# wdmwhh/MRefSR

Measured on AMD Instinct MI355X. Metric: 4x SR Mpix/sec, 5-ref 160x160->640x640; PSNR within 0.01 dB of ref, higher is better.
Workload: dtype f32

## Files before the change

mrefsr_amd/csrc/conv_wino4.hip:

```cpp
#include <cstdlib>
#include <type_traits>

#include "conv_wino_common.h"

namespace {
using namespace mrefsr_conv;
using namespace mrefsr_wino;

constexpr int NSLOT = 2;
constexpr int SLOT_BYTES = RAW_BYTES;
constexpr int RING_OFF = 0;
constexpr int RING_BYTES = 4 * 4 * 4096;
constexpr int X_LD = 32 + 4;
constexpr int X_BYTES = 4 * NTILE * X_LD * 4;
constexpr int SLOT_OFF = RING_OFF + RING_BYTES;
constexpr int BIAS_OFF = SLOT_OFF + NSLOT * SLOT_BYTES;
constexpr int SINK_OFF = BIAS_OFF + BIAS_MAX * 4;
constexpr int X_OFF = SINK_OFF + 256 * 16;
constexpr int LDS_BYTES = X_OFF + X_BYTES;
static_assert(LDS_BYTES <= 160 * 1024 && (RING_OFF & 4095) == 0 && (SLOT_OFF & 15) == 0 && (X_OFF & 15) == 0, "conv_wino4: LDS budget");
constexpr int NPD = 6, PROWS = 3;
static_assert(NPD * PROWS == PP && PROWS * PP * 4 <= 256, "conv_wino4: patch piece assignment");
constexpr unsigned int OOB = 0xffff0000u;

__device__ __forceinline__ f32x16 mma16(const u32x4 a, const u32x4 b, const f32x16 c)
{
    return __builtin_amdgcn_mfma_f32_32x32x16_f16(__builtin_bit_cast(f16x8, a), __builtin_bit_cast(f16x8, b), c, 0, 0, 0);
}

template <int I, int N, class F> __device__ __forceinline__ void sfor(F &&f)
{
    if constexpr (I < N) {
        f(std::integral_constant<int, I>{});
        sfor<I + 1, N>(f);
    }
}

__device__ __forceinline__ void bload16(f32x4 &dst, const unsigned int voff, const __amdgpu_buffer_rsrc_t srd, const unsigned int soff)
{
    asm volatile("s_nop 4\n\tbuffer_load_dwordx4 %0, %1, %2, %3 offen" : "=v"(dst) : "v"(voff), "s"(srd), "s"(soff) : "memory");
}
template <int N> __device__ __forceinline__ void vm_wait_p(f32x4 (&p)[NPD])
{
    asm volatile("s_waitcnt vmcnt(%6)" : "+v"(p[0]), "+v"(p[1]), "+v"(p[2]), "+v"(p[3]), "+v"(p[4]), "+v"(p[5]) : "n"(N) : "memory");
}
__device__ __forceinline__ void dma_group(const unsigned int m0v, const unsigned int voff, const void *sbase)
{
    asm volatile("s_mov_b32 m0, %0\n\ts_nop 0\n\tglobal_load_lds_dwordx4 %1, %2\n\tglobal_load_lds_dwordx4 %1, %2 offset:1024\n\t"
                 "global_load_lds_dwordx4 %1, %2 offset:2048\n\tglobal_load_lds_dwordx4 %1, %2 offset:3072"
                 : : "s"(m0v), "v"(voff), "s"(sbase) : "memory");
}
template <int OFF> __device__ __forceinline__ void dma_frag(const unsigned int m0v, const unsigned int voff, const void *sbase)
{
    if constexpr (OFF == 0)
        asm volatile("s_mov_b32 m0, %0\n\ts_nop 0\n\tglobal_load_lds_dwordx4 %1, %2" : : "s"(m0v), "v"(voff), "s"(sbase) : "memory");
    else
        asm volatile("global_load_lds_dwordx4 %0, %1 offset:%2" : : "v"(voff), "s"(sbase), "n"(OFF) : "memory");
}
template <int N> __device__ __forceinline__ void vm_wait() { asm volatile("s_waitcnt vmcnt(%0)" : : "n"(N) : "memory"); }

struct TState {
    f32x4 a[4], b[4], t[4], v[4];
};
template <int K>
__device__ __forceinline__ void top(TState &s, const unsigned char *const pa, const unsigned char *const pb, const float sr, u32x4 (&vh)[4], u32x4 (&vl)[4])
{
    constexpr int g0 = (K < 24 || (K >= 32 && K < 72)) ? 0 : 1;
    if constexpr (K < 8 || (K >= 24 && K < 32)) {
        constexpr int r = K < 8 ? K : K - 24, c = r >> 1;
        constexpr int co = ((c & 1) * RAW_CP + (c >> 1)) * 16 + g0 * (RAW_Q * 16);
        if constexpr (r & 1) s.b[c] = *reinterpret_cast<const f32x4 *>(pb + co);
        else s.a[c] = *reinterpret_cast<const f32x4 *>(pa + co);
    } else if constexpr ((K >= 8 && K < 24) || (K >= 72 && K < 88)) {
        constexpr int r = K < 24 ? K - 8 : K - 72, c = r >> 2, e = r & 3;
        s.t[c][e] = __builtin_fmaf(sr, s.b[c][e], s.a[c][e]);
    } else if constexpr ((K >= 32 && K < 48) || (K >= 88 && K < 104)) {
        constexpr int r = K < 48 ? K - 32 : K - 88, j = r >> 2, e = r & 3;
        if constexpr (j == 0) s.v[0][e] = s.t[0][e] - s.t[2][e];
        else if constexpr (j == 1) s.v[1][e] = s.t[1][e] + s.t[2][e];
        else if constexpr (j == 2) s.v[2][e] = s.t[2][e] - s.t[1][e];
        else s.v[3][e] = s.t[1][e] - s.t[3][e];
    } else {
        constexpr int r = K < 72 ? K - 48 : K - 104, u = r / 3, sub = r % 3, j = u >> 1, p = u & 1, w = 2 * g0 + p;
        if constexpr (sub == 0) vh[j][w] = pk_f16(s.v[j][2 * p], s.v[j][2 * p + 1]);
        else if constexpr (sub == 1) {
            unsigned int lo;
            asm("v_fma_mixlo_f16 %0, %1, -1.0, %2 op_sel_hi:[1,0,0]" : "=v"(lo) : "v"(vh[j][w]), "v"(s.v[j][2 * p]));
            vl[j][w] = lo;
        } else {
            unsigned int lo = vl[j][w];
            asm("v_fma_mixhi_f16 %0, %1, -1.0, %2 op_sel:[1,0,0] op_sel_hi:[1,0,0]" : "+v"(lo) : "v"(vh[j][w]), "v"(s.v[j][2 * p + 1]));
            vl[j][w] = lo;
        }
    }
}
constexpr int QA[24] = {4, 4, 6, 6, 6, 6, 5, 6, 5, 6, 6, 6, 4, 5, 4, 5, 5, 5, 5, 6, 5, 6, 6, 6};
constexpr int QB[24] = {4, 4, 5, 6, 6, 5, 5, 6, 5, 6, 6, 5, 5, 6, 5, 6, 6, 5, 5, 6, 5, 6, 5, 5};
constexpr int qsum(const int (&q)[24], const int n)
{
    int t = 0;
    for (int i = 0; i < n; ++i) t += q[i];
    return t;
}
static_assert(qsum(QA, 24) == 128 && qsum(QB, 24) == 128, "conv_wino4: every micro-operation of a transform is dealt exactly once");

#ifdef WINO_STAMP
constexpr int NSTAMP = 12;
__device__ unsigned long long g_wino4_stamp[1024][NSTAMP];
#define W4STAMP(i)                                                     \
    {                                                                 \
        const unsigned long long t_now = __builtin_readcyclecounter(); \
        st_acc[i] += t_now - t_last;                                  \
        t_last = t_now;                                               \
    }
#else
#define W4STAMP(i) {}
#endif

#ifndef W4_ABL
#define W4_ABL 0
#endif

template <int RES, bool NT, bool POOL, bool SCALED>
__global__ __launch_bounds__(256, 1) void conv_wino4_kernel(const ConvArgs A)
{
#ifdef WINO_STAMP
    unsigned long long st_acc[NSTAMP] = {0, 0, 0, 0, 0, 0, 0, 0, 0, 0, 0, 0}, t_last = __builtin_readcyclecounter();
#endif
    extern __shared__ __align__(16) unsigned char smem[];
    const int tid = threadIdx.x, lane = tid & 63, wi = __builtin_amdgcn_readfirstlane(tid >> 6);
    const int l31 = lane & 31, kh = lane >> 5;
    const int H = A.H, W = A.W;
    const int tiles_x = W / (2 * TT), tiles_y = H / (2 * TT);
    const int n_tiles = A.n_cb * tiles_x * tiles_y * A.wino_N, per = (n_tiles + 7) >> 3;
    const int band0 = (blockIdx.x & 7) * per, band1 = min(band0 + per, n_tiles), tstep = gridDim.x >> 3;
    int tile = band0 + (blockIdx.x >> 3);
    if (tile >= band1) return;
    for (int i = tid; i < A.n_cb * NB; i += 256)
        reinterpret_cast<float *>(smem + BIAS_OFF)[i] = (A.bias && i < A.Cout) ? A.bias[i] : 0.f;
    struct Tile { int n, cb, y0, x0; };
    auto decode = [&](const int lin) {
        Tile t;
        t.cb = lin % A.n_cb;
        int r = lin / A.n_cb;
        t.x0 = (r % tiles_x) * (2 * TT);
        r /= tiles_x;
        t.y0 = (r % tiles_y) * (2 * TT);
        t.n = r / tiles_y;
        return t;
    };
    const int n_ch = A.n_ch;

    f32x16 acc[4][2][2];

    f32x4 pf[NPD];
    const int p_q = tid & 3, p_py = (tid >> 2) / PP, p_px = (tid >> 2) - p_py * PP;
    const bool p_have = tid < PROWS * PP * 4;
    const unsigned int praw0 = p_have ? (unsigned int)(SLOT_OFF + (p_q * RAW_Q + p_py * RAW_RS + (p_px & 1) * RAW_CP + (p_px >> 1)) * 16) : (unsigned int)(SINK_OFF + tid * 16);
    const unsigned int praw_step = p_have ? (unsigned int)(PROWS * RAW_RS * 16) : 0u, praw_slot = p_have ? (unsigned int)SLOT_BYTES : 0u;
    Tile nxt = {0, 0, 0, 0};
    int rq_tile = tile, rq_ch = 0, rq_run = 0;
    int t_n = 0, t_y0 = 0, t_x0 = 0;
    __amdgpu_buffer_rsrc_t rq_srd = __builtin_amdgcn_make_buffer_rsrc(const_cast<float *>(A.x1), 0, 0, 0x00020000);
    unsigned int rq_soff = 0, rq_vo[NPD];
#pragma unroll
    for (int k = 0; k < NPD; ++k) rq_vo[k] = OOB;
    auto prepare = [&]() {
        const bool edge = rq_run == 0;
        const bool wrap = edge && rq_ch == n_ch;
        rq_tile += wrap ? tstep : 0;
        const int ch = wrap ? 0 : rq_ch;
        rq_ch = ch + 1;
        int run = rq_run - 1;
        unsigned int soff = rq_soff + KC * 4;
        if (edge) {
            if (ch == 0) {
                nxt = decode(rq_tile < band1 ? rq_tile : band0);
                t_n = rq_tile < band1 ? nxt.n : -1, t_y0 = nxt.y0, t_x0 = nxt.x0;
            }
            const bool first = ch < A.n_ch1;
            const int cl = first ? ch : ch - A.n_ch1, Cs = first ? A.C1 : A.C2;
            soff = (unsigned int)(cl * KC * 4);
            const int ld = first ? A.ld1 : A.ld2, nn = t_n < 0 ? 0 : t_n;
            const float *const img = first ? A.x1 + (size_t)(nn % A.N1) * H * W * A.ld1 : A.x2 + (size_t)(nn % A.N2) * H * W * A.ld2;
            const unsigned int bytes = __builtin_amdgcn_readfirstlane((unsigned int)((size_t)H * W * ld * 4));
            rq_srd = __builtin_amdgcn_make_buffer_rsrc(const_cast<void *>(scalar_ptr(img)), 0, bytes, 0x00020000);
            const int gy0 = t_y0 + p_py - 1, gx = t_x0 + p_px - 1;
            const bool cok = p_have & (t_n >= 0) & ((unsigned int)gx < (unsigned int)W) & (cl * KC + 4 * p_q < Cs);
            const unsigned int base = ((unsigned int)(gy0 * W + gx) * (unsigned int)ld + 4u * p_q) * 4u;
            const unsigned int step3 = (unsigned int)(PROWS * W * ld) * 4u;
#pragma unroll
            for (int k = 0; k < NPD; ++k)
                rq_vo[k] = (cok & ((unsigned int)(gy0 + k * PROWS) < (unsigned int)H)) ? base + (unsigned int)k * step3 : OOB;
            const int full = Cs / KC;
            run = cl < full ? full - 1 - cl : 0;
        }
        rq_run = __builtin_amdgcn_readfirstlane(run);
        rq_soff = __builtin_amdgcn_readfirstlane(soff);
    };
    auto request_piece = [&](const int k) { bload16(pf[k], rq_vo[k], rq_srd, __builtin_amdgcn_readfirstlane(rq_soff)); };
    float in_s = 1.f, oscale_in = A.out_scale;
    if constexpr (SCALED) {
        const float am = *A.in_amax;
        if (am > 1.0e-30f && am < 3.0e38f) {
            int e;
            (void)frexpf(am, &e);
            in_s = ldexpf(1.f, 12 - e);
            oscale_in = A.out_scale * ldexpf(1.f, e - 12);
        }
        in_s = __uint_as_float(__builtin_amdgcn_readfirstlane(__float_as_uint(in_s)));
    }
    auto store_piece = [&](const int slot, const int k) {
        f32x4 v = pf[k];
        if constexpr (SCALED) v[0] *= in_s, v[1] *= in_s, v[2] *= in_s, v[3] *= in_s;
        *reinterpret_cast<f32x4 *>(smem + praw0 + slot * praw_slot + k * praw_step) = v;
    };

    const int t_ra = wi == 0 ? 0 : (wi == 2 ? 2 : 1), t_rb = wi == 0 ? 2 : (wi == 1 ? 2 : (wi == 2 ? 1 : 3));
    const float t_sr = __uint_as_float(__builtin_amdgcn_readfirstlane(wi == 1 ? 0x3f800000u : 0xbf800000u));
    const unsigned int t_base = (unsigned int)(SLOT_OFF + ((2 * kh) * RAW_Q + (2 * (l31 >> 3)) * RAW_RS + (l31 & 7)) * 16);
    const unsigned int t_a = t_base + t_ra * RAW_RS * 16, t_b = t_base + t_rb * RAW_RS * 16;

    const unsigned int u_voff = (unsigned int)(l31 * KC + kh * 8) * 2u;
    const unsigned short *const u_wave = A.wp + (size_t)(wi * 4) * 2 * NB * KC;
    const unsigned int ring_w = (unsigned int)(RING_OFF + wi * 16384);
    const unsigned char *const frag_l = smem + ring_w + lane * 16;
    int uq_tile = tile, uq_left = 0;
    const unsigned char *u_s = nullptr;
    auto frag_cursor = [&]() {
        const bool edge = uq_left == 0;
        const unsigned char *nb = u_s + WCH_HALVES * 2;
        if (edge) {
            nb = reinterpret_cast<const unsigned char *>(scalar_ptr(u_wave + (size_t)nxt.cb * n_ch * WCH_HALVES));
        }
        u_s = nb;
        uq_tile += edge ? tstep : 0;
        uq_left = edge ? n_ch - 1 : uq_left - 1;
    };
    auto frag_dma = [&](const int j) { dma_group(ring_w + j * 4096, u_voff, u_s + j * 4096); };
    auto frag_dma1 = [&](const int j, auto pc) { dma_frag<decltype(pc)::value * 1024>(ring_w + j * 4096, u_voff, u_s + j * 4096); };
    auto frag_read = [&](const int j, const int ct, const int plane) {
        if constexpr (W4_ABL == 8) return u32x4{(unsigned int)(j + ct), (unsigned int)plane, 0x3c003c00u, 0x3c003c00u};
        else return *reinterpret_cast<const u32x4 *>(frag_l + j * 4096 + plane * 2048 + ct * 1024);
    };

    int sl = 0;
    prepare();
    Tile cur = nxt;
#pragma unroll
    for (int k = 0; k < NPD; ++k) request_piece(k);
    prepare();
    frag_cursor();
    vm_wait_p<0>(pf);
#pragma unroll
    for (int k = 0; k < NPD; ++k) store_piece(0, k);
#pragma unroll
    for (int k = 0; k < NPD; ++k) request_piece(k);
#pragma unroll
    for (int j = 0; j < 4; ++j) frag_dma(j);
    prepare();
    frag_cursor();
    __syncthreads();
    vm_wait_p<12>(pf);
    const float slope = __uint_as_float(__builtin_amdgcn_readfirstlane(__float_as_uint(!A.act ? 1.0f : A.slope_ptr ? *A.slope_ptr : A.slope)));
    u32x4 a0h[4], a0l[4];
    {
        TState ts;
        const unsigned char *const pa = smem + t_a, *const pb = smem + t_b;
        sfor<0, 128>([&](auto kc) { top<decltype(kc)::value>(ts, pa, pb, t_sr, a0h, a0l); });
    }
    float nonfin = 0.f;
    float oamx = 0.f;
    u32x4 ul[2], uh[2];
    ul[0] = frag_read(0, 0, 1), ul[1] = frag_read(0, 1, 1);

    auto step = [&](auto first_c) {
        constexpr bool first = decltype(first_c)::value;
        asm volatile("; W4MARK step_begin");
        u32x4 b1h[4], b1l[4];
        const int sl1 = sl ^ 1;
        {
            TState ts;
            const unsigned char *const pa = smem + t_a + sl * SLOT_BYTES + 8 * RAW_RS * 16;
            const unsigned char *const pb = smem + t_b + sl * SLOT_BYTES + 8 * RAW_RS * 16;
            sfor<0, 24>([&](auto mc) {
                constexpr int m = decltype(mc)::value, j = m / 6, k = m % 6, ct = k & 1, prod = k >> 1;
                if constexpr (m == 0) W4STAMP(0)
                if constexpr (m == 6) W4STAMP(1)
                if constexpr (m == 12) W4STAMP(2)
                if constexpr (m == 18) W4STAMP(3)
                if constexpr (k == 0) uh[0] = frag_read(j, 0, 0), uh[1] = frag_read(j, 1, 0);
                if constexpr (W4_ABL != 4) {
                    f32x16 z;
#pragma unroll
                    for (int e = 0; e < 16; ++e) z[e] = 0.f;
                    if constexpr (prod == 0) acc[j][0][ct] = mma16(ul[ct], a0h[j], first ? z : acc[j][0][ct]);
                    else if constexpr (prod == 1) acc[j][0][ct] = mma16(uh[ct], a0l[j], acc[j][0][ct]);
                    else acc[j][0][ct] = mma16(uh[ct], a0h[j], acc[j][0][ct]);
                } else {
                    asm volatile("" : : "v"(prod == 0 ? ul[ct] : uh[ct]), "v"(prod == 1 ? a0l[j] : a0h[j]));
                }
                if constexpr (W4_ABL != 3) sfor<qsum(QA, m), qsum(QA, m + 1)>([&](auto kc) { top<decltype(kc)::value>(ts, pa, pb, t_sr, b1h, b1l); });
                if constexpr (W4_ABL != 2 && W4_ABL != 7 && m >= 6 && m < 12) store_piece(sl1, m - 6);
                if constexpr (k == 4) {
                    if constexpr (j == 0) vm_wait<8>();
                    if constexpr (j == 1) vm_wait<4>();
                    if constexpr (j == 2) vm_wait<4>();
                    constexpr int jn = j == 3 ? 0 : j + 1;
                    ul[0] = frag_read(jn, 0, 1), ul[1] = frag_read(jn, 1, 1);
                }
                if constexpr (W4_ABL != 2 && W4_ABL != 7 && m >= 12 && m < 18) request_piece(m - 12);
                __builtin_amdgcn_sched_barrier(0);
            });
        }
        W4STAMP(4)
        {
            TState ts;
            const unsigned char *const pa = smem + t_a + sl1 * SLOT_BYTES;
            const unsigned char *const pb = smem + t_b + sl1 * SLOT_BYTES;
            sfor<0, 24>([&](auto mc) {
                constexpr int m = decltype(mc)::value, j = m / 6, k = m % 6, ct = k & 1, prod = k >> 1;
                if constexpr (k == 0) uh[0] = frag_read(j, 0, 0), uh[1] = frag_read(j, 1, 0);
                if constexpr (W4_ABL != 4) {
                    f32x16 z;
#pragma unroll
                    for (int e = 0; e < 16; ++e) z[e] = 0.f;
                    if constexpr (prod == 0) acc[j][1][ct] = mma16(ul[ct], b1h[j], first ? z : acc[j][1][ct]);
                    else if constexpr (prod == 1) acc[j][1][ct] = mma16(uh[ct], b1l[j], acc[j][1][ct]);
                    else acc[j][1][ct] = mma16(uh[ct], b1h[j], acc[j][1][ct]);
                } else {
                    asm volatile("" : : "v"(prod == 0 ? ul[ct] : uh[ct]), "v"(prod == 1 ? b1l[j] : b1h[j]));
                }
                if constexpr (m == 0) {
                    if constexpr (W4_ABL != 6) __syncthreads();
                    W4STAMP(5)
                    __builtin_amdgcn_sched_barrier(0);
                }
                if constexpr (m == 12) W4STAMP(6)
                if constexpr (W4_ABL != 3) sfor<qsum(QB, m), qsum(QB, m + 1)>([&](auto kc) { top<decltype(kc)::value>(ts, pa, pb, t_sr, a0h, a0l); });
                if constexpr (k == 4 && j < 3) ul[0] = frag_read(j + 1, 0, 1), ul[1] = frag_read(j + 1, 1, 1);
                if constexpr (m == 22) {
                    vm_wait_p<10>(pf);
                    ul[0] = frag_read(0, 0, 1), ul[1] = frag_read(0, 1, 1);
                }
                if constexpr (W4_ABL != 1 && W4_ABL != 7 && k >= 2) frag_dma1(j, std::integral_constant<int, k - 2>{});
                __builtin_amdgcn_sched_barrier(0);
            });
        }
        asm volatile("; W4MARK step_cursors");
        W4STAMP(7)
        prepare();
        frag_cursor();
        sl = sl1;
        asm volatile("; W4MARK step_end");
        W4STAMP(8)
    };

    for (;;) {
        const int tile_n = tile + tstep;
        const bool more = tile_n < band1;
        W4STAMP(10)
        step(std::true_type{});
        for (int s = 1; s < n_ch; ++s) step(std::false_type{});

        asm volatile("; W4MARK fast_begin");
        const int cb = cur.cb, n = cur.n, y0 = cur.y0, x0 = cur.x0;
        float *const xb = reinterpret_cast<float *>(smem + X_OFF);
        const int Cout = A.Cout;
        const float oscale = oscale_in;
        int tid_e = tid;
        asm volatile("" : "+v"(tid_e));
        const int c4 = (tid_e & 7) * 4, T0 = tid_e >> 3;
        float *const xrow0 = xb + ((size_t)wi * NTILE + (tid_e & 31)) * X_LD + 4 * ((tid_e >> 5) & 1);
        auto rd = [](const float &a) {
            float v;
            asm volatile("v_accvgpr_read_b32 %0, %1" : "=v"(v) : "a"(a));
            return v;
        };
        auto publish = [&](const int hc, const int b) {
#pragma unroll
            for (int t = 0; t < 2; ++t) {
                float *const xrow = xrow0 + t * 32 * X_LD;
#pragma unroll
                for (int qd = 0; qd < 4; ++qd) {
                    float z[4];
#pragma unroll
                    for (int r = 0; r < 4; ++r) {
                        const int e = 4 * qd + r;
                        if (b == 0) {
                            const float m0 = rd(acc[0][t][hc][e]), m1 = rd(acc[1][t][hc][e]), m2 = rd(acc[2][t][hc][e]);
                            z[r] = m0 + m1 + m2;
                        } else {
                            const float m1 = rd(acc[1][t][hc][e]), m2 = rd(acc[2][t][hc][e]), m3 = rd(acc[3][t][hc][e]);
                            z[r] = m1 + (-m2 - m3);
                        }
                    }
                    *reinterpret_cast<float4 *>(xrow + 8 * qd) = make_float4(z[0], z[1], z[2], z[3]);
                }
            }
        };
        auto gather = [&](const int T, float4 (&y)[2]) {
            float4 z[4];
#pragma unroll
            for (int i = 0; i < 4; ++i) z[i] = *reinterpret_cast<const float4 *>(xb + ((size_t)i * NTILE + T) * X_LD + c4);
            y[0] = make_float4(z[0].x + z[1].x + z[2].x, z[0].y + z[1].y + z[2].y, z[0].z + z[1].z + z[2].z, z[0].w + z[1].w + z[2].w);
            y[1] = make_float4(z[1].x - z[2].x - z[3].x, z[1].y - z[2].y - z[3].y, z[1].z - z[2].z - z[3].z, z[1].w - z[2].w - z[3].w);
        };
        {
            constexpr bool pooled = POOL;
            const int Ho = pooled ? H >> 1 : H, Wo = pooled ? W >> 1 : W, yo = pooled ? y0 >> 1 : y0, xo = pooled ? x0 >> 1 : x0;
            const int ld_r = RES == 2 ? Cout : A.ld_res;
            const __amdgpu_buffer_rsrc_t srd_o = __builtin_amdgcn_make_buffer_rsrc(
                const_cast<void *>(scalar_ptr(A.out + ((size_t)(n * Ho + yo) * Wo + xo) * A.ld_out + cb * NB)), 0, 0xffffffffu, 0x00020000);
            const float *const rbase = RES == 1 ? A.residual + ((size_t)(n * H + y0) * W + x0) * ld_r + cb * NB
                                     : RES == 2 ? A.pre + ((size_t)((n % A.pre_N) * H + y0) * W + x0) * ld_r + cb * NB : A.out;
            const __amdgpu_buffer_rsrc_t srd_r = __builtin_amdgcn_make_buffer_rsrc(const_cast<void *>(scalar_ptr(rbase)), 0, 0xffffffffu, 0x00020000);
            const int pstep = pooled ? 1 : 2;
            const unsigned int vo_o = (unsigned int)(((pstep * (T0 >> 3)) * Wo + pstep * (T0 & 7)) * A.ld_out + c4) * 4u;
            const unsigned int vo_r = (unsigned int)(((2 * (T0 >> 3)) * W + 2 * (T0 & 7)) * ld_r + c4) * 4u;
            const unsigned int row_o = (unsigned int)(Wo * A.ld_out) * 4u, row_r = (unsigned int)(W * ld_r) * 4u;
            constexpr int aux = NT ? 2 : 0;
            if constexpr (W4_ABL == 5) {
#pragma unroll
                for (int j = 0; j < 4; ++j)
#pragma unroll
                    for (int t = 0; t < 4; ++t) nonfin = __builtin_fmaf(rd(acc[j][t >> 1][t & 1][0]), 0.f, nonfin);
            }
#pragma unroll
            for (int hc = 0; hc < (W4_ABL == 5 ? 0 : 2); ++hc) {
                const float4 bv = *reinterpret_cast<const float4 *>(smem + BIAS_OFF + (cb * NB + hc * 32 + c4) * 4);
                float4 pool[2];
#pragma unroll
                for (int b = 0; b < 2; ++b) {
                    if (hc | b) __syncthreads();
                    f32x4 rq[2][2];
                    if constexpr (RES != 0) {
#pragma unroll
                        for (int it = 0; it < 2; ++it)
#pragma unroll
                            for (int a = 0; a < 2; ++a) {
                                const unsigned int so = (unsigned int)(8 * it + a) * row_r + (unsigned int)(b * ld_r + hc * 32) * 4u;
                                rq[it][a] = __builtin_bit_cast(f32x4, __builtin_amdgcn_raw_buffer_load_b128(srd_r, vo_r, so, aux));
                            }
                    }
                    publish(hc, b);
                    __syncthreads();
#pragma unroll
                    for (int it = 0; it < 2; ++it) {
                        __builtin_amdgcn_sched_barrier(0);
                        float4 y[2];
                        gather(T0 + 32 * it, y);
                        if constexpr (pooled) {
                            nonfin = __builtin_fmaf(y[0].x + y[1].x, 0.f, nonfin);
                            float4 m = make_float4(fmaxf(y[0].x, y[1].x), fmaxf(y[0].y, y[1].y), fmaxf(y[0].z, y[1].z), fmaxf(y[0].w, y[1].w));
                            if (b == 0) {
                                pool[it] = m;
                            } else {
                                m = make_float4(fmaxf(m.x, pool[it].x), fmaxf(m.y, pool[it].y), fmaxf(m.z, pool[it].z), fmaxf(m.w, pool[it].w));
                                float4 v = make_float4(m.x * oscale + bv.x, m.y * oscale + bv.y, m.z * oscale + bv.z, m.w * oscale + bv.w);
                                nonfin = __builtin_fmaf(v.x, 0.f, nonfin);
                                v.x = v.x > 0.f ? v.x : v.x * slope, v.y = v.y > 0.f ? v.y : v.y * slope;
                                v.z = v.z > 0.f ? v.z : v.z * slope, v.w = v.w > 0.f ? v.w : v.w * slope;
                                const unsigned int so = (unsigned int)(4 * it) * row_o + (unsigned int)(hc * 32) * 4u;
                                oamx = fmaxf(fmaxf(fmaxf(oamx, fabsf(v.x)), fabsf(v.y)), fmaxf(fabsf(v.z), fabsf(v.w)));
                                __builtin_amdgcn_raw_buffer_store_b128(__builtin_bit_cast(u32x4, f32x4{v.x, v.y, v.z, v.w}), srd_o, vo_o, so, aux);
                            }
                        } else {
#pragma unroll
                            for (int a = 0; a < 2; ++a) {
                                float4 v = y[a];
                                v.x = v.x * oscale + bv.x, v.y = v.y * oscale + bv.y, v.z = v.z * oscale + bv.z, v.w = v.w * oscale + bv.w;
                                nonfin = __builtin_fmaf(v.x, 0.f, nonfin);
                                if constexpr (RES == 2) v.x += rq[it][a][0], v.y += rq[it][a][1], v.z += rq[it][a][2], v.w += rq[it][a][3];
                                v.x = v.x > 0.f ? v.x : v.x * slope, v.y = v.y > 0.f ? v.y : v.y * slope;
                                v.z = v.z > 0.f ? v.z : v.z * slope, v.w = v.w > 0.f ? v.w : v.w * slope;
                                if constexpr (RES == 1) v.x += rq[it][a][0], v.y += rq[it][a][1], v.z += rq[it][a][2], v.w += rq[it][a][3];
                                const unsigned int so = (unsigned int)(8 * it + a) * row_o + (unsigned int)(b * A.ld_out + hc * 32) * 4u;
                                oamx = fmaxf(fmaxf(fmaxf(oamx, fabsf(v.x)), fabsf(v.y)), fmaxf(fabsf(v.z), fabsf(v.w)));
                                __builtin_amdgcn_raw_buffer_store_b128(__builtin_bit_cast(u32x4, f32x4{v.x, v.y, v.z, v.w}), srd_o, vo_o, so, aux);
                            }
                        }
                    }
                }
            }
        }
        asm volatile("; W4MARK fast_end");
        W4STAMP(9)
        if (!more) break;
        tile = tile_n;
        cur = nxt;
    }
    vm_wait_p<0>(pf);
#pragma unroll
    for (int k = 0; k < NPD; ++k) asm volatile("" ::"v"(pf[k]) : "memory");
#pragma unroll
    for (int j = 0; j < 4; ++j) asm volatile("" ::"v"(a0h[j]), "v"(a0l[j]) : "memory");
    if (A.range_flag && !(nonfin == nonfin)) atomicOr(A.range_flag, 1);
    if (A.stat_amax) {
#pragma unroll
        for (int o = 32; o > 0; o >>= 1) oamx = fmaxf(oamx, __shfl_xor(oamx, o, 64));
        if (lane == 0 && oamx > 0.f && oamx < 3.0e38f && __float_as_uint(oamx) > __builtin_nontemporal_load(A.stat_amax)) atomicMax(A.stat_amax, __float_as_uint(oamx));
    }
#ifdef WINO_STAMP
    W4STAMP(10)
    st_acc[11] = 1;
    if (lane == 0)
        for (int i = 0; i < NSTAMP; ++i) atomicAdd(&g_wino4_stamp[(blockIdx.x * 4 + wi) & 1023][i], st_acc[i]);
#endif
}

}

namespace mrefsr_conv {

bool wino4_serves(const ConvArgs &a)
{
    if ((a.H & 15) || (a.W & 15) || (a.Cout & 63) || (a.ld_out & 3) || (a.ld1 & 3) || (a.C1 & 3) || (a.x2 && ((a.ld2 & 3) || (a.C2 & 3)))) return false;
    if (a.epilogue == 1) return !a.residual && !a.pre;
    if (a.epilogue != 0) return false;
    if (a.residual && a.pre) return false;
    if (a.residual && (a.ld_res & 3)) return false;
    return true;
}

int wino4_launch(const ConvArgs &b, int blocks_cu, hipStream_t stream)
{
    const int res = b.residual ? 1 : b.pre ? 2 : 0;
    const bool pool = b.epilogue == 1, nt = b.stream_out != 0;
    const bool sc = b.in_amax != nullptr;
    using K = void (*)(const ConvArgs);
    static const K table[4][2][2] = {
        {{conv_wino4_kernel<0, false, false, false>, conv_wino4_kernel<0, false, false, true>},
         {conv_wino4_kernel<0, true, false, false>, conv_wino4_kernel<0, true, false, true>}},
        {{conv_wino4_kernel<1, false, false, false>, conv_wino4_kernel<1, false, false, true>},
         {conv_wino4_kernel<1, true, false, false>, conv_wino4_kernel<1, true, false, true>}},
        {{conv_wino4_kernel<2, false, false, false>, conv_wino4_kernel<2, false, false, true>},
         {conv_wino4_kernel<2, true, false, false>, conv_wino4_kernel<2, true, false, true>}},
        {{conv_wino4_kernel<0, false, true, false>, conv_wino4_kernel<0, false, true, true>},
         {conv_wino4_kernel<0, true, true, false>, conv_wino4_kernel<0, true, true, true>}}};
    const int ki = pool ? 3 : res;
    const K kern = table[ki][nt ? 1 : 0][sc ? 1 : 0];
    static unsigned long long attr[16] = {0, 0, 0, 0, 0, 0, 0, 0, 0, 0, 0, 0, 0, 0, 0, 0};
    if (mrefsr::first_use_on_device(attr[(ki * 2 + (nt ? 1 : 0)) * 2 + (sc ? 1 : 0)]))
        (void)hipFuncSetAttribute(reinterpret_cast<const void *>(kern), hipFuncAttributeMaxDynamicSharedMemorySize, LDS_BYTES);
    hipLaunchKernelGGL(kern, dim3(blocks_cu), dim3(256), LDS_BYTES, stream, b);
    return mrefsr::check_launch("conv_wino4");
}

}

#ifdef WINO_STAMP
MREFSR_EXPORT int mrefsr_dbg_wino4_stamps(unsigned long long *out12)
{
    static unsigned long long h[1024][NSTAMP];
    if (hipDeviceSynchronize() != hipSuccess) return mrefsr::fail(MREFSR_E_LAUNCH, "wino4_stamps: sync failed");
    if (hipMemcpyFromSymbol(h, HIP_SYMBOL(g_wino4_stamp), sizeof(h)) != hipSuccess) return mrefsr::fail(MREFSR_E_LAUNCH, "wino4_stamps: read failed");
    for (int i = 0; i < NSTAMP; ++i) out12[i] = 0;
    for (int s = 0; s < 1024; ++s)
        for (int i = 0; i < NSTAMP; ++i) out12[i] += h[s][i], h[s][i] = 0;
    if (hipMemcpyToSymbol(HIP_SYMBOL(g_wino4_stamp), h, sizeof(h)) != hipSuccess) return mrefsr::fail(MREFSR_E_LAUNCH, "wino4_stamps: reset failed");
    return 0;
}
#endif
```

Before: 16.19.

## Software-pipeline Winograd output epilogue: precompute column folds and prefetch residuals

Restructures the epilogue of the Winograd conv kernel. The AGPR reads and column fold for the next half-channel group are computed while the current group's LDS gather is in flight, and residual loads are issued one phase ahead. The aim is to hide AGPR-read, LDS and global-load latency behind the barrier-separated publish/gather phases. The cost is more live VGPRs for the prefolded values and prefetched residuals, which may raise register pressure or cause spills.

```diff
diff --git a/mrefsr_amd/csrc/conv_wino4.hip b/mrefsr_amd/csrc/conv_wino4.hip
--- a/mrefsr_amd/csrc/conv_wino4.hip
+++ b/mrefsr_amd/csrc/conv_wino4.hip
@@ -367,7 +367,6 @@
         const int cb = cur.cb, n = cur.n, y0 = cur.y0, x0 = cur.x0;
         float *const xb = reinterpret_cast<float *>(smem + X_OFF);
         const int Cout = A.Cout;
-        const float oscale = oscale_in;
         int tid_e = tid;
         asm volatile("" : "+v"(tid_e));
         const int c4 = (tid_e & 7) * 4, T0 = tid_e >> 3;
@@ -377,34 +376,22 @@
             asm volatile("v_accvgpr_read_b32 %0, %1" : "=v"(v) : "a"(a));
             return v;
         };
-        auto publish = [&](const int hc, const int b) {
-#pragma unroll
-            for (int t = 0; t < 2; ++t) {
-                float *const xrow = xrow0 + t * 32 * X_LD;
-#pragma unroll
-                for (int qd = 0; qd < 4; ++qd) {
-                    float z[4];
-#pragma unroll
-                    for (int r = 0; r < 4; ++r) {
-                        const int e = 4 * qd + r;
-                        if (b == 0) {
-                            const float m0 = rd(acc[0][t][hc][e]), m1 = rd(acc[1][t][hc][e]), m2 = rd(acc[2][t][hc][e]);
-                            z[r] = m0 + m1 + m2;
-                        } else {
-                            const float m1 = rd(acc[1][t][hc][e]), m2 = rd(acc[2][t][hc][e]), m3 = rd(acc[3][t][hc][e]);
-                            z[r] = m1 + (-m2 - m3);
-                        }
-                    }
-                    *reinterpret_cast<float4 *>(xrow + 8 * qd) = make_float4(z[0], z[1], z[2], z[3]);
-                }
+        auto colfold = [&](const int hc, const int t, f32x2 (&z0)[8], f32x2 (&z1)[8]) {
+#pragma unroll
+            for (int p = 0; p < 8; ++p) {
+                const int e = 2 * p;
+                const f32x2 m0 = f32x2{rd(acc[0][t][hc][e]), rd(acc[0][t][hc][e + 1])}, m1 = f32x2{rd(acc[1][t][hc][e]), rd(acc[1][t][hc][e + 1])};
+                const f32x2 m2 = f32x2{rd(acc[2][t][hc][e]), rd(acc[2][t][hc][e + 1])}, m3 = f32x2{rd(acc[3][t][hc][e]), rd(acc[3][t][hc][e + 1])};
+                z0[p] = f32x2{m0[0] + m1[0] + m2[0], m0[1] + m1[1] + m2[1]};
+                z1[p] = f32x2{m1[0] + (-m2[0] - m3[0]), m1[1] + (-m2[1] - m3[1])};
             }
         };
-        auto gather = [&](const int T, float4 (&y)[2]) {
-            float4 z[4];
-#pragma unroll
-            for (int i = 0; i < 4; ++i) z[i] = *reinterpret_cast<const float4 *>(xb + ((size_t)i * NTILE + T) * X_LD + c4);
-            y[0] = make_float4(z[0].x + z[1].x + z[2].x, z[0].y + z[1].y + z[2].y, z[0].z + z[1].z + z[2].z, z[0].w + z[1].w + z[2].w);
-            y[1] = make_float4(z[1].x - z[2].x - z[3].x, z[1].y - z[2].y - z[3].y, z[1].z - z[2].z - z[3].z, z[1].w - z[2].w - z[3].w);
+        auto publish = [&](const f32x2 (&z)[2][8]) {
+#pragma unroll
+            for (int t = 0; t < 2; ++t)
+#pragma unroll
+                for (int qd = 0; qd < 4; ++qd)
+                    *reinterpret_cast<f32x4 *>(xrow0 + t * 32 * X_LD + 8 * qd) = f32x4{z[t][2 * qd][0], z[t][2 * qd][1], z[t][2 * qd + 1][0], z[t][2 * qd + 1][1]};
         };
         {
             constexpr bool pooled = POOL;
@@ -426,61 +413,102 @@
 #pragma unroll
                     for (int t = 0; t < 4; ++t) nonfin = __builtin_fmaf(rd(acc[j][t >> 1][t & 1][0]), 0.f, nonfin);
             }
+            f32x4 rqn[2][2];
+            auto request = [&](const int hc, const int b) {
+                if constexpr (RES != 0) {
+#pragma unroll
+                    for (int it = 0; it < 2; ++it)
+#pragma unroll
+                        for (int a = 0; a < 2; ++a) {
+                            const unsigned int so = (unsigned int)(8 * it + a) * row_r + (unsigned int)(b * ld_r + hc * 32) * 4u;
+                            rqn[it][a] = __builtin_bit_cast(f32x4, __builtin_amdgcn_raw_buffer_load_b128(srd_r, vo_r, so, aux));
+                        }
+                }
+            };
+            request(0, 0);
+            f32x2 zc[2][2][8];
+            if constexpr (W4_ABL != 5) colfold(0, 0, zc[0][0], zc[1][0]), colfold(0, 1, zc[0][1], zc[1][1]);
+            const float oscale = oscale_in;
 #pragma unroll
             for (int hc = 0; hc < (W4_ABL == 5 ? 0 : 2); ++hc) {
-                const float4 bv = *reinterpret_cast<const float4 *>(smem + BIAS_OFF + (cb * NB + hc * 32 + c4) * 4);
-                float4 pool[2];
+                const f32x4 bv = *reinterpret_cast<const f32x4 *>(smem + BIAS_OFF + (cb * NB + hc * 32 + c4) * 4);
+                f32x2 zn[2][2][8];
+                float pool[2][4];
 #pragma unroll
                 for (int b = 0; b < 2; ++b) {
                     if (hc | b) __syncthreads();
+                    publish(zc[b]);
+                    __syncthreads();
                     f32x4 rq[2][2];
                     if constexpr (RES != 0) {
 #pragma unroll
-                        for (int it = 0; it < 2; ++it)
-#pragma unroll
-                            for (int a = 0; a < 2; ++a) {
-                                const unsigned int so = (unsigned int)(8 * it + a) * row_r + (unsigned int)(b * ld_r + hc * 32) * 4u;
-                                rq[it][a] = __builtin_bit_cast(f32x4, __builtin_amdgcn_raw_buffer_load_b128(srd_r, vo_r, so, aux));
-                            }
+                        for (int it = 0; it < 2; ++it) rq[it][0] = rqn[it][0], rq[it][1] = rqn[it][1];
+                        if (!(hc & b)) request(hc + b, b ^ 1);
                     }
-                    publish(hc, b);
-                    __syncthreads();
+                    f32x4 zr[2][4];
+#pragma unroll
+                    for (int it = 0; it < 2; ++it)
+#pragma unroll
+                        for (int i = 0; i < 4; ++i) zr[it][i] = *reinterpret_cast<const f32x4 *>(xb + ((size_t)i * NTILE + T0 + 32 * it) * X_LD + c4);
+                    __builtin_amdgcn_sched_barrier(0);
+                    if (hc == 0) {
+                        colfold(1, b, zn[0][b], zn[1][b]);
+                        __builtin_amdgcn_sched_barrier(0);
+                    }
 #pragma unroll
                     for (int it = 0; it < 2; ++it) {
-                        __builtin_amdgcn_sched_barrier(0);
-                        float4 y[2];
-                        gather(T0 + 32 * it, y);
+                        f32x4 y[2];
+#pragma unroll
+                        for (int c = 0; c < 4; ++c) {
+                            y[0][c] = zr[it][0][c] + zr[it][1][c] + zr[it][2][c];
+                            y[1][c] = zr[it][1][c] - zr[it][2][c] - zr[it][3][c];
+                        }
                         if constexpr (pooled) {
-                            nonfin = __builtin_fmaf(y[0].x + y[1].x, 0.f, nonfin);
-                            float4 m = make_float4(fmaxf(y[0].x, y[1].x), fmaxf(y[0].y, y[1].y), fmaxf(y[0].z, y[1].z), fmaxf(y[0].w, y[1].w));
+                            nonfin = __builtin_fmaf(y[0][0] + y[1][0], 0.f, nonfin);
+                            f32x4 m;
+#pragma unroll
+                            for (int c = 0; c < 4; ++c) m[c] = fmaxf(y[0][c], y[1][c]);
                             if (b == 0) {
-                                pool[it] = m;
+#pragma unroll
+                                for (int c = 0; c < 4; ++c) pool[it][c] = m[c];
                             } else {
-                                m = make_float4(fmaxf(m.x, pool[it].x), fmaxf(m.y, pool[it].y), fmaxf(m.z, pool[it].z), fmaxf(m.w, pool[it].w));
-                                float4 v = make_float4(m.x * oscale + bv.x, m.y * oscale + bv.y, m.z * oscale + bv.z, m.w * oscale + bv.w);
-                                nonfin = __builtin_fmaf(v.x, 0.f, nonfin);
-                                v.x = v.x > 0.f ? v.x : v.x * slope, v.y = v.y > 0.f ? v.y : v.y * slope;
-                                v.z = v.z > 0.f ? v.z : v.z * slope, v.w = v.w > 0.f ? v.w : v.w * slope;
+                                f32x4 v;
+#pragma unroll
+                                for (int c = 0; c < 4; ++c) v[c] = fmaxf(m[c], pool[it][c]) * oscale + bv[c];
+                                nonfin = __builtin_fmaf(v[0], 0.f, nonfin);
+#pragma unroll
+                                for (int c = 0; c < 4; ++c) v[c] = v[c] > 0.f ? v[c] : v[c] * slope;
                                 const unsigned int so = (unsigned int)(4 * it) * row_o + (unsigned int)(hc * 32) * 4u;
-                                oamx = fmaxf(fmaxf(fmaxf(oamx, fabsf(v.x)), fabsf(v.y)), fmaxf(fabsf(v.z), fabsf(v.w)));
-                                __builtin_amdgcn_raw_buffer_store_b128(__builtin_bit_cast(u32x4, f32x4{v.x, v.y, v.z, v.w}), srd_o, vo_o, so, aux);
+                                oamx = fmaxf(fmaxf(fmaxf(oamx, fabsf(v[0])), fabsf(v[1])), fmaxf(fabsf(v[2]), fabsf(v[3])));
+                                __builtin_amdgcn_raw_buffer_store_b128(__builtin_bit_cast(u32x4, v), srd_o, vo_o, so, aux);
                             }
                         } else {
 #pragma unroll
                             for (int a = 0; a < 2; ++a) {
-                                float4 v = y[a];
-                                v.x = v.x * oscale + bv.x, v.y = v.y * oscale + bv.y, v.z = v.z * oscale + bv.z, v.w = v.w * oscale + bv.w;
-                                nonfin = __builtin_fmaf(v.x, 0.f, nonfin);
-                                if constexpr (RES == 2) v.x += rq[it][a][0], v.y += rq[it][a][1], v.z += rq[it][a][2], v.w += rq[it][a][3];
-                                v.x = v.x > 0.f ? v.x : v.x * slope, v.y = v.y > 0.f ? v.y : v.y * slope;
-                                v.z = v.z > 0.f ? v.z : v.z * slope, v.w = v.w > 0.f ? v.w : v.w * slope;
-                                if constexpr (RES == 1) v.x += rq[it][a][0], v.y += rq[it][a][1], v.z += rq[it][a][2], v.w += rq[it][a][3];
+                                f32x4 v;
+#pragma unroll
+                                for (int c = 0; c < 4; ++c) v[c] = y[a][c] * oscale + bv[c];
+                                nonfin = __builtin_fmaf(v[0], 0.f, nonfin);
+#pragma unroll
+                                for (int c = 0; c < 4; ++c) {
+                                    if constexpr (RES == 2) v[c] += rq[it][a][c];
+                                    v[c] = v[c] > 0.f ? v[c] : v[c] * slope;
+                                    if constexpr (RES == 1) v[c] += rq[it][a][c];
+                                }
                                 const unsigned int so = (unsigned int)(8 * it + a) * row_o + (unsigned int)(b * A.ld_out + hc * 32) * 4u;
-                                oamx = fmaxf(fmaxf(fmaxf(oamx, fabsf(v.x)), fabsf(v.y)), fmaxf(fabsf(v.z), fabsf(v.w)));
-                                __builtin_amdgcn_raw_buffer_store_b128(__builtin_bit_cast(u32x4, f32x4{v.x, v.y, v.z, v.w}), srd_o, vo_o, so, aux);
+                                oamx = fmaxf(fmaxf(fmaxf(oamx, fabsf(v[0])), fabsf(v[1])), fmaxf(fabsf(v[2]), fabsf(v[3])));
+                                __builtin_amdgcn_raw_buffer_store_b128(__builtin_bit_cast(u32x4, v), srd_o, vo_o, so, aux);
                             }
                         }
                     }
+                }
+                if (hc == 0) {
+#pragma unroll
+                    for (int b = 0; b < 2; ++b)
+#pragma unroll
+                        for (int t = 0; t < 2; ++t)
+#pragma unroll
+                            for (int p = 0; p < 8; ++p) zc[b][t][p] = zn[b][t][p];
                 }
             }
         }
```

Result: faster. 16.42, median of 6 (+1.5%).
